# yyyyyxie/textflux

Hardware: AMD Instinct MI355X
Metric: images/sec (whole node), 1024x1024 30-step FLUX-Fill (higher is better)
Workload: dtype bf16

## Files before the change

textflux_amd/csrc/attention_w4.hip:

```cpp
#include <mutex>
#include <type_traits>

#include "common.h"
#include "launch.h"

namespace tfx {

namespace {
constexpr int W4_KV = 64, W4_HD = 128;
constexpr int W4_VT = W4_KV * 256;
constexpr int W4_KROW = 272;
constexpr int W4_KT = W4_KV * W4_KROW;
constexpr int W4_NBUF = 3;
constexpr int W4_KBASE = W4_NBUF * W4_VT;
constexpr int W4_PROW = 132;
__device__ __forceinline__ int w4_part_off(int r, int col) {
  return ((((r >> 5) * 4 + (col >> 5)) * 4 + ((col >> 3) & 3)) * 64 + ((col >> 2) & 1) * 32 + (r & 31)) * 4;
}
constexpr int W4_PART_LM = 256 * 128;
constexpr float W4_THR = 4.0f;
constexpr float W4_BIG = 64.0f;
typedef __attribute__((address_space(3))) s16x4 lds_s16x4;
typedef __attribute__((ext_vector_type(8))) short s16x8;
typedef __attribute__((ext_vector_type(2))) __bf16 bf2_t;
template <int V>
using IC = std::integral_constant<int, V>;
}

constexpr int ATT_LDS_W4 = W4_NBUF * (W4_VT + W4_KT);

#define W4_GAP() __builtin_amdgcn_sched_barrier(0)
#ifndef W4_ABL
#define W4_ABL 0
#endif
#define W4_DRAIN_MFMA()                                                                                                 \
  asm volatile("s_nop 15\n\ts_nop 15\n\ts_nop 15\n\ts_nop 15\n\ts_nop 15\n\ts_nop 15\n\ts_nop 15\n\ts_nop 15\n\t"      \
               "s_nop 15\n\ts_nop 15\n\ts_nop 15\n\ts_nop 15\n\ts_nop 15\n\ts_nop 15\n\ts_nop 15\n\ts_nop 15\n\t"      \
               "s_nop 15\n\ts_nop 15\n\ts_nop 15\n\ts_nop 15\n\ts_nop 15\n\ts_nop 15\n\ts_nop 15\n\ts_nop 15" ::: "memory")

#ifndef W4_NO_TOUCH
#define W4_TOUCH(acc)                                                                  \
  do {                                                                                 \
    const int t_ = __builtin_amdgcn_readfirstlane(__float_as_int((acc)[0]));           \
    asm volatile("" ::"s"(t_));                                                        \
  } while (0)
#else
#define W4_TOUCH(acc) do { } while (0)
#endif

__device__ __forceinline__ void w4_mfma_s0(f32x16& d, const bf16x8& k, const bf16x8& q) {
  f32x16 z;
#pragma unroll
  for (int r = 0; r < 16; ++r) z[r] = 0.f;
  d = __builtin_amdgcn_mfma_f32_32x32x16_bf16(k, q, z, 0, 0, 0);
}
__device__ __forceinline__ void w4_mfma_s(f32x16& d, const bf16x8& k, const bf16x8& q) {
  d = __builtin_amdgcn_mfma_f32_32x32x16_bf16(k, q, d, 0, 0, 0);
}
__device__ __forceinline__ void w4_mfma_o(f32x16& d, const bf16x8& v, const u32x4& p) {
  d = __builtin_amdgcn_mfma_f32_32x32x16_bf16(v, __builtin_bit_cast(bf16x8, p), d, 0, 0, 0);
}
__device__ __forceinline__ void w4_mfma_l(f32x16& d, const bf16x8& ones, const u32x4& p) {
  d = __builtin_amdgcn_mfma_f32_32x32x16_bf16(ones, __builtin_bit_cast(bf16x8, p), d, 0, 0, 0);
}
__device__ __forceinline__ float w4_max7(float a, float b, float c, float d, float e, float f, float g) {
  float r;
  asm("v_max3_f32 %0, %1, %2, %3\n\tv_max3_f32 %0, %0, %4, %5\n\tv_max3_f32 %0, %0, %6, %7"
      : "=&v"(r) : "v"(a), "v"(b), "v"(c), "v"(d), "v"(e), "v"(f), "v"(g));
  return r;
}
__device__ __forceinline__ float w4_max4(float a, float b, float c, float d) {
  float r;
  asm("v_max3_f32 %0, %1, %2, %3\n\tv_max_f32 %0, %0, %4" : "=&v"(r) : "v"(a), "v"(b), "v"(c), "v"(d));
  return r;
}
__device__ __forceinline__ float w4_max(float a, float b) {
  float r;
  asm("v_max_f32 %0, %1, %2" : "=v"(r) : "v"(a), "v"(b));
  return r;
}
__device__ __forceinline__ void w4_dot2c(float& l, uint32_t p) {
  asm volatile("v_dot2c_f32_bf16 %0, 0x3f803f80, %1" : "+v"(l) : "v"(p));
}
__device__ __forceinline__ uint32_t w4_cvt_pk(float lo, float hi) {
  uint32_t r;
  asm volatile("v_cvt_pk_bf16_f32 %0, %1, %2" : "=v"(r) : "v"(lo), "v"(hi));
  return r;
}
#ifdef TFX_BENCH
__device__ unsigned long long* g_w4_timers = nullptr;
#define W4_STAMP(i) do { if (wave == 0) w4_stamp[i] = __builtin_amdgcn_s_memtime(); } while (0)
#else
#define W4_STAMP(i) ((void)0)
#endif
constexpr int W4_SK_MIN = 4;
__host__ __device__ __forceinline__ int w4_sk_bound(int c, int group, int share, int nkv, int total) {
  if (c >= group) return total;
  int p = c * share;
  if (p >= total) return total;
  const int r = p % nkv;
  if (r < W4_SK_MIN) p -= r;
  else if (r > nkv - W4_SK_MIN) p += nkv - r;
  return p < total ? p : total;
}

template <int MODE>
__global__ __launch_bounds__(256, 1) void attn_w4_kernel(const bf16_t* Q, const bf16_t* __restrict__ Kp,
                                                         const bf16_t* __restrict__ Vp, bf16_t* O, int64_t ldq, int64_t ldk,
                                                         int64_t ldv, int64_t ldo, int64_t q_bs, int64_t k_bs, int64_t v_bs,
                                                         int64_t o_bs, int H, int N, int nqb, float scale_log2e, int nfull,
                                                         int nparts, int nsplit, int xsplit, float* part, int T_items, int sk_group,
                                                         int sk_share) {
  extern __shared__ __attribute__((aligned(16))) char smem[];
  constexpr bool LV = MODE == 1 || MODE == 2, LZ = MODE >= 2, NOREF = MODE == 4, FT = LV || NOREF;
  const int tid = threadIdx.x, lane = tid & 63;
  const int wave = __builtin_amdgcn_readfirstlane(tid >> 6);
  const int hi = lane >> 5, l31 = lane & 31;
  int bid = blockIdx.x;
  int kpart = -1, ptile = 0, qblk, h, b;
  int item = 0, item_step = 0, item_end = 0;
  int sk_lo = 0, sk_hi = 0, sk_base = 0, sk_slot0 = 0, sk_u = 0, sk_nunits = 0, sk_nwhole = 0, sk_full = 0, sk_cu = 0, sk_tfirst = 0;
  const int nkv_all = (N + W4_KV - 1) / W4_KV;
  auto sk_unit = [&](int u, int& it, int& ts, int& te) __attribute__((always_inline)) {
    if (u < sk_nwhole) {
      it = sk_base + sk_cu + u * sk_group; ts = 0; te = nkv_all;
    } else {
      const int ti = sk_tfirst + (u - sk_nwhole);
      it = sk_base + sk_full + ti; ts = max(sk_lo - ti * nkv_all, 0); te = min(sk_hi - ti * nkv_all, nkv_all);
    }
  };
  int ts = 0, te = nkv_all;
  if (sk_share > 0) {
    const int L = (bid & 7) * (gridDim.x >> 3) + (bid >> 3);
    const int sample = L / sk_group;
    sk_cu = L - sample * sk_group;
    if (sample >= nfull) return;
    sk_full = (T_items / sk_group) * sk_group;
// ... 850 lines not shown
  if (hipDeviceGetAttribute(&s.cus, hipDeviceAttributeMultiprocessorCount, dev) != hipSuccess || s.cus < 8) s.cus = 256;
  if (hipMalloc((void**)&s.part, (size_t)W4_PART_TILES * 256 * W4_PROW * sizeof(float)) != hipSuccess) {
    (void)hipGetLastError();
    return nullptr;
  }
  g_w4_scr[g_w4_nscr] = s;
  return &g_w4_scr[g_w4_nscr++];
}

int attention_w4_release() {
  std::lock_guard<std::mutex> lk(g_w4_mu);
  if (g_w4_nscr == 0) return 0;
  (void)hipDeviceSynchronize();
  int cur = 0;
  (void)hipGetDevice(&cur);
  for (int i = 0; i < g_w4_nscr; ++i) {
    (void)hipSetDevice(g_w4_scr[i].dev);
    (void)hipDeviceSynchronize();
    (void)hipFree(g_w4_scr[i].part);
  }
  (void)hipSetDevice(cur);
  (void)hipGetLastError();
  g_w4_nscr = 0;
  return 0;
}

int attention_w4_prepare(hipStream_t st) {
  if (!g_w4_split) return 0;
  return w4_scratch(st, true) ? 0 : fail("attention: cannot allocate the tail-split scratch");
}

static int g_w4_streamk = 1;
void set_attention_streamk(int v) { g_w4_streamk = v; }
static int g_w4_persist = 1;
void set_attention_persistent(int v) { g_w4_persist = v; }
static int g_w4_grid() {
  static int grid = 0;
  if (!grid) {
    int dev = 0, cus = 0;
    (void)hipGetDevice(&dev);
    if (hipDeviceGetAttribute(&cus, hipDeviceAttributeMultiprocessorCount, dev) != hipSuccess || cus < 8) cus = 256;
    grid = cus & ~7;
  }
  return grid;
}

#ifdef TFX_BENCH
extern "C" void tfx_bench_attn_timers(unsigned long long* dev) {
  (void)hipMemcpyToSymbol(HIP_SYMBOL(g_w4_timers), &dev, sizeof(dev));
}
#endif

template <int MODE>
static int w4_launch(const AttnArgs& a, hipStream_t st, unsigned grid, int nqb, int nfull, int nparts, int nsplit, int xsplit, float* part,
                     int sk_group, int sk_share) {
  static bool attr_set = false;
  const void* fn = (const void*)attn_w4_kernel<MODE>;
  if (!attr_set) {
    hipFuncAttributes fa;
    if (hipFuncGetAttributes(&fa, fn) != hipSuccess) return fail("attention: no attn_w4_kernel<%d> in this build", MODE);
    (void)hipGetLastError();
    if (fa.localSizeBytes != 0)
      return fail("attention: attn_w4_kernel<%d> spills %zu bytes per lane -- attention_w4.hip must be compiled with "
                  "-mllvm -amdgpu-mfma-vgpr-form", MODE, (size_t)fa.localSizeBytes);
    if (hipFuncSetAttribute(fn, hipFuncAttributeMaxDynamicSharedMemorySize, ATT_LDS_W4 + ((W4_ABL & 256) ? 4096 : 0)) != hipSuccess)
      return fail("attention: cannot raise dynamic LDS limit to %d bytes", ATT_LDS_W4);
    attr_set = true;
  }
  int T_items = 0;
  if (sk_share > 0) {
    T_items = a.H * nqb;
    nfull = a.B;
    grid = (unsigned)g_w4_grid();
  } else if (g_w4_persist && nsplit == 1 && (int)grid > g_w4_grid()) {
    T_items = (int)grid;
    grid = (unsigned)g_w4_grid();
  }
  attn_w4_kernel<MODE><<<grid, 256, ATT_LDS_W4 + ((W4_ABL & 256) ? 4096 : 0), st>>>((const bf16_t*)a.q, (const bf16_t*)a.k, (const bf16_t*)a.v, (bf16_t*)a.o, a.ldq,
                                                       a.ldk, a.ldv, a.ldo, a.q_bstride, a.k_bstride, a.v_bstride, a.o_bstride, a.H,
                                                       a.N, nqb, a.scale * 1.4426950408889634f, nfull, nparts, nsplit, xsplit, part, T_items, sk_group, sk_share);
  return 0;
}

int joint_attention_w4(const AttnArgs& a, hipStream_t st, int mode) {
  const int nqb = (a.N + 255) / 256;
  const int T = a.B * a.H * nqb;
  int nfull = T, nsplit = 1, nparts = 0, xsplit = 0;
  float* part = nullptr;
  if (g_w4_split) {
    hipStreamCaptureStatus cs = hipStreamCaptureStatusNone;
    const bool capturing = !(hipStreamIsCapturing(st, &cs) == hipSuccess && cs == hipStreamCaptureStatusNone);
    (void)hipGetLastError();
    if (const W4Scratch* sc = w4_scratch(st, !capturing)) {
      const int C = sc->cus, tail = T % C, nkv = (a.N + W4_KV - 1) / W4_KV;
      const int m = (tail + a.B - 1) / a.B;
      if (tail && T >= C && m * a.B * 2 <= C + 8 && nkv >= 48 && m < a.H * nqb && m * a.B * 2 <= W4_PART_TILES) {
        xsplit = m; nsplit = 2; nfull = T - m * a.B; nparts = m * a.B * 2; part = sc->part;
      }
    }
  }
  int sk_group = 0, sk_share = 0;
  if (g_w4_streamk && g_w4_persist && nsplit == 1 && a.workspace && a.B <= g_w4_grid()) {
    const int C = g_w4_grid(), nkv = (a.N + W4_KV - 1) / W4_KV, Tp = a.H * nqb, group = C / a.B;
    const int full = (Tp / group) * group, R = Tp - full;
    const int share = R ? (R * nkv + group - 1) / group : 0;
    const int64_t need = (int64_t)2 * a.B * group * 256 * W4_PROW * (int64_t)sizeof(float);
    const float F = 7.f, M = 20.f;
    const float t_whole = (float)(full / group) * ((float)nkv + F);
    const float t_now = t_whole + (float)nkv + F, t_sk = t_whole + (float)share + ((float)share / (float)nkv + 1.f) * F + M;
// ... 30 lines not shown
```

textflux_amd/csrc/capi.cpp:

```cpp
#include "../../include/textflux_hip.h"

#include <cstring>

#include "launch.h"

using namespace tfx;

namespace {

inline hipStream_t S(tfx_stream s) { return (hipStream_t)s; }
inline const uint16_t* bf(const void* p) { return (const uint16_t*)p; }
inline uint16_t* bf(void* p) { return (uint16_t*)p; }

struct Gemm {
  GemmArgs a;
  const tfx_linear* lin;
  Gemm(const void* A, int64_t lda, int64_t abs_, const tfx_linear& l, int64_t ldw, void* C, int64_t ldc, int64_t cbs,
       int M, int N, int K, int batch) : lin(&l) {
    a = GemmArgs();
    a.A = A; a.lda = lda; a.a_bstride = abs_;
    a.W = l.w; a.ldw = ldw; a.bias = l.b;
    a.C = C; a.ldc = ldc; a.c_bstride = cbs;
    a.M = M; a.N = N; a.K = K; a.batch = batch;
    a.epilogue = EPI_BIAS;
// ... 558 lines not shown
int tfx_gather_rows(const void* table, const int64_t* ids, void* out, int64_t n, int32_t D, int64_t vocab, tfx_stream stream) {
  if (!table || !ids || !out) return fail("tfx_gather_rows: null pointer");
  return gather_rows(table, ids, out, n, D, vocab, S(stream));
}
int tfx_add_into_f32(float* x, const void* y, int64_t n, int32_t mode, tfx_stream stream) {
  if (!x || !y) return fail("tfx_add_into_f32: null pointer");
  return add_into_f32(x, y, n, mode, S(stream));
}
int tfx_mul_act(const void* a, int64_t lda, const void* b, int64_t ldb, void* out, int64_t ldo, int64_t rows, int32_t cols,
                int32_t mode, tfx_stream stream) {
  if (!a || !out) return fail("tfx_mul_act: null pointer");
  return mul_act(a, lda, b, ldb, out, ldo, rows, cols, mode, S(stream));
}

int tfx_set_option(const char* name, int value) {
  if (!name) return fail("tfx_set_option: null name");
  if (!std::strcmp(name, "attention_waves")) {
    if (value == 0) { set_attention_waves(0); return 0; }
    if (value != 4 && value != 8 && value != 9 && value != 10 && value != 12 && value != 16 && value != 20 && !(value >= 30 && value <= 34) && value != 40)
      return fail("tfx_set_option: attention_waves must be 4, 8, 9 (128 keys per barrier), 10 / 12 (matrix-pipe softmax, 8 / 4 waves), 16 (ping-pong), 20 (half-tile pipelined), 30 .. 34 (one wave per SIMD, 32x32x16 MFMA: 30 bookkeeping on the matrix pipe -- or no reference at all when the call carries an admissible score bound -- / 31 row sums on the VALU / 32 = 31 + lazy reference offset / 33 = 30 + lazy reference offset / 34 = no reference with a score bound, else 33) or 40 (one wave per SIMD, 16x16x32 MFMA)");
#ifndef TFX_BENCH
    if (value != 30 && value != 34)
      return fail("tfx_set_option: attention_waves %d is a bench-only kernel (libtextflux_hip_bench.so, `make bench`); the product library "
                  "carries 30 (the default) and 34", value);
#endif
    set_attention_waves(value);
    return 0;
  }
  if (!std::strcmp(name, "gemm_group_m")) { set_gemm_group_m(value); return 0; }
  if (!std::strcmp(name, "attention_tail_split")) { set_attention_tail_split(value); return 0; }
  if (!std::strcmp(name, "attention_use_bound")) { set_attention_use_bound(value); return 0; }
  if (!std::strcmp(name, "attention_persistent")) { set_attention_persistent(value); return 0; }
  if (!std::strcmp(name, "attention_streamk")) { set_attention_streamk(value); return 0; }
  if (!std::strcmp(name, "gemm_place")) { set_gemm_place(value); return 0; }
  if (!std::strcmp(name, "gemm_waves")) {
#ifndef TFX_BENCH
    if (value != 8 && value != 0) return fail("tfx_set_option: gemm_waves 4 (gemm4w_kernel) is bench-only (libtextflux_hip_bench.so, `make bench`)");
#endif
    set_gemm_waves(value);
    return 0;
  }
  if (!std::strcmp(name, "gemm_group_streams")) { g_group_streams = value; return 0; }
  if (!std::strcmp(name, "ln_joint")) { g_ln_joint = value; return 0; }
  if (!std::strcmp(name, "ln_prefetch")) { set_ln_prefetch(value); return 0; }
  if (!std::strcmp(name, "fp8_fuse_qkn")) { g_fp8_fuse_qkn = value; return 0; }
  if (!std::strcmp(name, "gemm_splitk")) { set_gemm_splitk(value); return 0; }
  if (!std::strcmp(name, "attention_ablation")) { set_attention_ablation(value); return 0; }
  return fail("tfx_set_option: unknown option '%s'", name);
}

int tfx_debug_attention_timing(void* buf) { set_attention_debug(buf); return 0; }

int tfx_mfma_peak_probe(const void* operands, int64_t operand_bytes, int32_t fp8, int32_t ktiles, double* flops, tfx_stream stream) {
  return mfma_peak_probe(operands, operand_bytes, fp8, ktiles, flops, S(stream));
}

int tfx_prof_enable(int on) { prof_enable(on); return 0; }
int tfx_prof_collect(int kind, double* total_ms, double* total_flops, int* launches) {
  if (kind < 0 || kind > 2) return fail("tfx_prof_collect: kind must be 0 (gemm), 1 (attention) or 2 (fp8 gemm)");
  return prof_collect(kind, total_ms, total_flops, launches);
}

static inline int64_t align256(int64_t v) { return (v + 255) & ~(int64_t)255; }
int tfx_workspace_layout(int32_t B, int32_t Sn, int32_t T, int32_t D, int32_t flags, int64_t* off, int64_t* gemm_ws_bytes) {
  if (B <= 0 || Sn <= 0 || T < 0 || D <= 0 || !off) return fail("tfx_workspace_layout: bad arguments");
  const int64_t N = (int64_t)Sn + T, hid = align256(B * N * D * 2), y = align256(B * N * 7 * (int64_t)D * 2);
// ... 102 lines not shown
```

textflux_amd/csrc/launch.h:

```cpp
#pragma once
#include <hip/hip_runtime.h>
#include <stdint.h>

namespace tfx {

int fail(const char* fmt, ...);
int check_launch(const char* what);
const char* last_error();

void prof_enable(int on);
bool prof_on();
bool prof_on(hipStream_t st);
void prof_begin(int kind, double flops, hipStream_t st);
void prof_end(int kind, hipStream_t st);
int prof_collect(int kind, double* total_ms, double* total_flops, int* launches);

enum Epilogue : int {
  EPI_BIAS = 0,
  EPI_BIAS_GELU = 1,
  EPI_BIAS_GATE_RES = 2,
  EPI_BIAS_RES = 3,
};

struct GemmArgs {
// ... 24 lines not shown
void set_gemm_place(int v);
void set_gemm_waves(int v);
void set_gemm_splitk(int v);
int gemm_bf16(const GemmArgs& a, hipStream_t st);
bool gemm_qkn_ok(const GemmArgs& a);
bool gemm_fp8_qkn_ok(const GemmArgs& a);
int gemm_bf16_variant(const GemmArgs& a, int variant, hipStream_t st);
int gemm_bf16_f32out(const GemmArgs& a, hipStream_t st);
int mfma_peak_probe(const void* operands, int64_t operand_bytes, int fp8, int ktiles, double* flops, hipStream_t st);
int gemm_fp8(const GemmArgs& a, hipStream_t st);
int ln_modulate_fp8(const void* x, void* q8, float* q8_scale, const void* shift, const void* scale, int64_t mod_bstride,
                    int rows_per_batch, int batch, int D, int64_t ldx, int64_t x_bstride, int64_t ldq, int64_t q_bstride,
                    int64_t s_bstride, float eps, hipStream_t st);
int quantize_rows_fp8(const void* x, int64_t ldx, int64_t x_bstride, void* out, int64_t ldo, int64_t o_bstride, float* scale,
                      int64_t s_bstride, int rows, int batch, int K, hipStream_t st);

struct AttnArgs {
  const void* q; const void* k; const void* v; void* o;
  int64_t ldq, ldk, ldv, ldo;
  int64_t q_bstride, k_bstride, v_bstride, o_bstride;
  int B, H, N;
  float scale;
  float score_bound = 0.f;
  void* workspace = nullptr;
  int64_t workspace_bytes = 0;
};
int joint_attention(const AttnArgs& a, hipStream_t st);
int joint_attention_hp(const AttnArgs& a, hipStream_t st);
int joint_attention_w16(const AttnArgs& a, hipStream_t st);
int attention_w4_release();
int attention_w4_prepare(hipStream_t st);
void set_attention_tail_split(int v);
int joint_attention_w4(const AttnArgs& a, hipStream_t st, int mode);
void set_attention_ablation(int a);
void set_attention_use_bound(int v);
int attention_mode_counts(int64_t* counts, int n, int reset);
void attention_note_streamk();
int blend_edge(const void* a, int64_t a_bs, int64_t a_ts, int64_t a_us, void* b, int64_t b_bs, int64_t b_ts, int64_t b_us, int batch,
               int extent, int len, int C, hipStream_t st);
int gate_residual(const void* x, int64_t ldx, int64_t x_bs, const void* gate, int64_t gate_bs, const void* res, int64_t ldr, int64_t r_bs,
                  void* out, int64_t ldo, int64_t o_bs, int rows, int batch, int D, hipStream_t st);
void set_attention_streamk(int v);
void set_attention_persistent(int v);
void set_attention_debug(void* p);
void set_attention_waves(int nw);

int groupnorm_silu_nhwc(const void* x, void* out, const void* gamma, const void* beta, float* stats_ws, int B,
                        int64_t HW, int C, int groups, float eps, bool silu, hipStream_t st);
void set_ln_prefetch(int v);
int ln_modulate_split(const void* x, void* out, const void* shift, const void* scale, const void* shift2, const void* scale2,
                      int split_row, int64_t mod_bstride, int rows_per_batch, int batch, int D, int64_t ldx, int64_t x_bstride, int64_t ldo,
                      int64_t o_bstride, float eps, hipStream_t st);
int ln_modulate(const void* x, void* out, const void* shift, const void* scale, int64_t mod_bstride,
                int rows_per_batch, int batch, int D, int64_t ldx, int64_t x_bstride, int64_t ldo,
                int64_t o_bstride, float eps, hipStream_t st);
int layernorm_affine(const void* x, void* out, const void* gamma, const void* beta, int64_t rows, int D, int64_t ldx, int64_t ldo,
                     float eps, hipStream_t st);
int rmsnorm_rope(void* buf, int64_t ld, int64_t bstride, int q_off, int k_off, int H, int Ntok, int T, int B,
                 const void* wq_img, const void* wk_img, const void* wq_txt, const void* wk_txt, const float* cosT,
                 const float* sinT, float eps, hipStream_t st);
int sched_step(bool amo, const void* v, void* x, void* xin, int64_t ldxin, int C, int64_t rows, const float* coef,
               const int* step_ptr, int step, const float* noise, hipStream_t st);
int timestep_embedding(const float* t, void* out, int n, hipStream_t st);
int silu_bf16(const void* a, void* out, int64_t n, hipStream_t st);
int add_bf16(const void* a, const void* b, void* out, int64_t n, hipStream_t st);
int scatter_cols(const void* src, void* dst, int64_t rows, int C, int64_t ld, int col0, hipStream_t st);
// ... 32 lines not shown
```

Baseline: 0.5871.

## Add register-resident fixed-reference attention kernel for the no-rescale mode

Adds a separate attention kernel that is used for MODE 4 (the no-reference-max path) when there is no tail split. It keeps a dedicated software-pipelined schedule: raw v_exp with no running max or rescale, row sums accumulated with v_add instead of an MFMA or dot2c, next-item Q prefetched into registers, and K/V staged through registers into a triple LDS buffer. Shared constants and helpers move to a common header. The aim is fewer instructions per tile in the exp/sum stage and better MFMA/VALU interleaving, at the cost of a second large hand-scheduled kernel to maintain.

```diff
diff --git a/textflux_amd/csrc/attention_rf.hip b/textflux_amd/csrc/attention_rf.hip
--- /dev/null
+++ b/textflux_amd/csrc/attention_rf.hip
@@ -0,0 +1,438 @@
+#include "attention_w4.h"
+#include "launch.h"
+
+namespace tfx {
+
+#ifdef TFX_BENCH
+__device__ unsigned long long* g_rf_timers = nullptr;
+#define RF_STAMP(i) do { if (wave == 0) rf_stamp[i] = __builtin_amdgcn_s_memtime(); } while (0)
+#else
+#define RF_STAMP(i) ((void)0)
+#endif
+
+__device__ __forceinline__ float rf_exp(float x) {
+  asm volatile("v_exp_f32 %0, %0" : "+v"(x));
+  return x;
+}
+__device__ __forceinline__ void rf_add(float& l, float x) { asm volatile("v_add_f32 %0, %0, %1" : "+v"(l) : "v"(x)); }
+
+__global__ __launch_bounds__(256, 1) void attn_rf_kernel(const bf16_t* Q, const bf16_t* __restrict__ Kp, const bf16_t* __restrict__ Vp,
+                                                         bf16_t* O, int64_t ldq, int64_t ldk, int64_t ldv, int64_t ldo, int64_t q_bs,
+                                                         int64_t k_bs, int64_t v_bs, int64_t o_bs, int H, int N, int nqb, float scale_log2e,
+                                                         int nfull, float* part, int T_items, int sk_group, int sk_share) {
+  extern __shared__ __attribute__((aligned(16))) char smem[];
+  const int tid = threadIdx.x, lane = tid & 63;
+  const int wave = __builtin_amdgcn_readfirstlane(tid >> 6);
+  const int hi = lane >> 5, l31 = lane & 31;
+  int bid = blockIdx.x;
+  int qblk, h, b;
+  int item = 0, item_step = 0, item_end = 0;
+  int sk_lo = 0, sk_hi = 0, sk_base = 0, sk_slot0 = 0, sk_u = 0, sk_nunits = 0, sk_nwhole = 0, sk_full = 0, sk_cu = 0, sk_tfirst = 0;
+  const int nkv_all = (N + W4_KV - 1) / W4_KV;
+  auto sk_unit = [&](int u, int& it, int& ts, int& te) __attribute__((always_inline)) {
+    if (u < sk_nwhole) {
+      it = sk_base + sk_cu + u * sk_group; ts = 0; te = nkv_all;
+    } else {
+      const int ti = sk_tfirst + (u - sk_nwhole);
+      it = sk_base + sk_full + ti; ts = max(sk_lo - ti * nkv_all, 0); te = min(sk_hi - ti * nkv_all, nkv_all);
+    }
+  };
+  int ts = 0, te = nkv_all;
+  if (sk_share > 0) {
+    const int L = (bid & 7) * (gridDim.x >> 3) + (bid >> 3);
+    const int sample = L / sk_group;
+    sk_cu = L - sample * sk_group;
+    if (sample >= nfull) return;
+    sk_full = (T_items / sk_group) * sk_group;
+    sk_nwhole = sk_full / sk_group;
+    const int total = (T_items - sk_full) * nkv_all;
+    sk_lo = w4_sk_bound(sk_cu, sk_group, sk_share, nkv_all, total);
+    sk_hi = w4_sk_bound(sk_cu + 1, sk_group, sk_share, nkv_all, total);
+    sk_tfirst = sk_lo / nkv_all;
+    sk_nunits = sk_nwhole + (sk_hi > sk_lo ? (sk_hi - 1) / nkv_all - sk_tfirst + 1 : 0);
+    if (sk_nunits == 0) return;
+    sk_base = sample * T_items;
+    sk_slot0 = 2 * L;
+    sk_unit(0, item, ts, te);
+  } else if (T_items > 0) {
+    const int nwg = gridDim.x, q = T_items >> 3, r = T_items & 7, xcd = bid & 7, slot = bid >> 3;
+    const int xs = xcd < r ? xcd * (q + 1) : r * (q + 1) + (xcd - r) * q, xc = q + (xcd < r ? 1 : 0);
+    if (slot >= xc) return;
+    item = xs + slot;
+    item_step = nwg >> 3;
+    item_end = xs + xc;
+  } else {
+    const int nwg = gridDim.x, q = nwg >> 3, r = nwg & 7, xcd = bid & 7, k = bid >> 3;
+    item = (xcd < r ? xcd * (q + 1) : r * (q + 1) + (xcd - r) * q) + k;
+  }
+  qblk = item % nqb;
+  h = (item / nqb) % H;
+  b = item / (nqb * H);
+  bf16x8 qn[2][8];
+  bool have_pref = false;
+  u32x4 kreg[4], vreg[4];
+#ifdef TFX_BENCH
+  unsigned long long rf_stamp[4] = {0, 0, 0, 0}, rf_sum[4] = {0, 0, 0, 0};
+#endif
+  for (;;) {
+  RF_STAMP(0);
+  bool has_next = item + item_step < item_end;
+  int item2 = item + item_step, ts2 = 0;
+  if (sk_share > 0) {
+    int te2;
+    has_next = sk_u + 1 < sk_nunits;
+    if (has_next) sk_unit(sk_u + 1, item2, ts2, te2);
+  }
+  const int qblk2 = item2 % nqb, h2 = (item2 / nqb) % H, b2 = item2 / (nqb * H);
+  const bf16_t* Qb = Q + b * q_bs + h * W4_HD;
+  const bf16_t* Kb = Kp + b * k_bs + h * W4_HD;
+  const bf16_t* Vb = Vp + b * v_bs + h * W4_HD;
+  bf16_t* Ob = O + b * o_bs + h * W4_HD;
+  int Nk = N;
+  int pslot = -1;
+  if (sk_share > 0) {
+    if (ts > 0) pslot = sk_slot0;
+    else if (te < nkv_all) pslot = sk_slot0 + 1;
+    Nk = min(N, te * W4_KV) - ts * W4_KV;
+    Kb += (int64_t)ts * W4_KV * ldk;
+    Vb += (int64_t)ts * W4_KV * ldv;
+  }
+
+  bf16x8 qf[2][8];
+#pragma unroll
+  for (int qb = 0; qb < 2; ++qb) {
+    const int qrow = qblk * 256 + wave * 64 + qb * 32 + l31;
+    const int rc = qrow < N ? qrow : N - 1;
+    if (have_pref) {
+#pragma unroll
+      for (int s = 0; s < 8; ++s) qf[qb][s] = qn[qb][s];
+    } else {
+#pragma unroll
+      for (int s = 0; s < 8; ++s) qf[qb][s] = *reinterpret_cast<const bf16x8*>(Qb + (int64_t)rc * ldq + s * 16 + hi * 8);
+    }
+  }
+  auto load_qn = [&]() __attribute__((always_inline)) {
+    const bf16_t* Qb2 = Q + b2 * q_bs + h2 * W4_HD;
+#pragma unroll
+    for (int qb = 0; qb < 2; ++qb) {
+      const int r2 = qblk2 * 256 + wave * 64 + qb * 32 + l31;
+      const int rc = r2 < N ? r2 : N - 1;
+#pragma unroll
+      for (int s = 0; s < 8; ++s) qn[qb][s] = *reinterpret_cast<const bf16x8*>(Qb2 + (int64_t)rc * ldq + s * 16 + hi * 8);
+    }
+  };
+  __builtin_amdgcn_sched_barrier(0);
+  auto convert_q = [&]() __attribute__((always_inline)) {
+#pragma unroll
+    for (int qb = 0; qb < 2; ++qb)
+#pragma unroll
+      for (int s = 0; s < 8; ++s) {
+#pragma unroll
+        for (int e = 0; e < 8; ++e) qf[qb][s][e] = (__bf16)((float)qf[qb][s][e] * scale_log2e);
+        asm volatile("" : "+a"(qf[qb][s]));
+      }
+  };
+
+  const int nkv = (Nk + W4_KV - 1) / W4_KV;
+  const int ldk2 = (int)ldk * 2, ldv2 = (int)ldv * 2;
+  const auto rsK = __builtin_amdgcn_make_buffer_rsrc((void*)Kb, 0, (int)((uint32_t)(Nk - 1) * (uint32_t)ldk2 + 256u), 0x00020000);
+  const auto rsV = __builtin_amdgcn_make_buffer_rsrc((void*)Vb, 0, (int)((uint32_t)(Nk - 1) * (uint32_t)ldv2 + 256u), 0x00020000);
+  const auto rsK2 = __builtin_amdgcn_make_buffer_rsrc((void*)(Kp + b2 * k_bs + h2 * W4_HD + (int64_t)ts2 * W4_KV * ldk), 0,
+                                                      (int)((uint32_t)(N - 1 - ts2 * W4_KV) * (uint32_t)ldk2 + 256u), 0x00020000);
+  const auto rsV2 = __builtin_amdgcn_make_buffer_rsrc((void*)(Vp + b2 * v_bs + h2 * W4_HD + (int64_t)ts2 * W4_KV * ldv), 0,
+                                                      (int)((uint32_t)(N - 1 - ts2 * W4_KV) * (uint32_t)ldv2 + 256u), 0x00020000);
+  auto rsKs = rsK, rsVs = rsV;
+  auto load_piece = [&](int j, int ko, int vo, auto Ic, bool k_side) __attribute__((always_inline)) {
+    constexpr int i = decltype(Ic)::value;
+    if (k_side)
+      kreg[i] = __builtin_bit_cast(u32x4, __builtin_amdgcn_raw_buffer_load_b128(rsKs, ko, (j * W4_KV + 16 * i) * ldk2, 0));
+    else
+      vreg[i] = __builtin_bit_cast(u32x4, __builtin_amdgcn_raw_buffer_load_b128(rsVs, vo, (j * W4_KV + 16 * i) * ldv2, 0));
+  };
+  auto stage_offsets = [&](int& ko, int& vo) __attribute__((always_inline)) {
+    int te_ = tid;
+    asm volatile("" : "+v"(te_));
+    ko = (int)__umul24(te_ >> 4, ldk2) + (te_ & 15) * 16;
+    vo = (int)__umul24(te_ >> 4, ldv2) + (te_ & 15) * 16;
+  };
+  auto load_tile = [&](int j) __attribute__((always_inline)) {
+    int ko, vo;
+    stage_offsets(ko, vo);
+    load_piece(j, ko, vo, IC<0>{}, true); load_piece(j, ko, vo, IC<0>{}, false); load_piece(j, ko, vo, IC<1>{}, true); load_piece(j, ko, vo, IC<1>{}, false);
+    load_piece(j, ko, vo, IC<2>{}, true); load_piece(j, ko, vo, IC<2>{}, false); load_piece(j, ko, vo, IC<3>{}, true); load_piece(j, ko, vo, IC<3>{}, false);
+  };
+  auto write_piece = [&](int buf, auto Ic, bool k_side) __attribute__((always_inline)) {
+    constexpr int i = decltype(Ic)::value;
+    const int kr = tid >> 4, ch = tid & 15;
+    if (k_side)
+      *reinterpret_cast<u32x4*>(smem + W4_KBASE + buf * W4_KT + kr * W4_KROW + ch * 16 + i * 16 * W4_KROW) = kreg[i];
+    else
+      *reinterpret_cast<u32x4*>(smem + buf * W4_VT + kr * 256 + ((((ch >> 2) ^ (kr & 3)) << 6) | ((ch & 3) << 4)) + i * 16 * 256) = vreg[i];
+  };
+  auto write_tile = [&](int buf) __attribute__((always_inline)) {
+    write_piece(buf, IC<0>{}, true); write_piece(buf, IC<0>{}, false); write_piece(buf, IC<1>{}, true); write_piece(buf, IC<1>{}, false);
+    write_piece(buf, IC<2>{}, true); write_piece(buf, IC<2>{}, false); write_piece(buf, IC<3>{}, true); write_piece(buf, IC<3>{}, false);
+  };
+  const char* rK = smem + W4_KBASE + l31 * W4_KROW + hi * 16;
+  const int vi = lane & 15;
+  const char* rV[4];
+#pragma unroll
+  for (int db = 0; db < 4; ++db)
+    rV[db] = smem + (4 * hi + (vi >> 2)) * 256 + 32 * ((lane >> 4) & 1) + (vi & 3) * 8 + ((db ^ ((vi >> 2) & 3)) << 6);
+  auto kread = [&](int koff, int s) __attribute__((always_inline)) -> bf16x8 {
+    return *reinterpret_cast<const bf16x8*>(rK + koff + s * 32);
+  };
+  auto vread = [&](int voff, int ks, int db) __attribute__((always_inline)) -> bf16x8 {
+    const char* va = rV[db] + voff + ks * 16 * 256;
+    const s16x4 lo = __builtin_amdgcn_ds_read_tr16_b64_v4i16((lds_s16x4*)(va));
+    const s16x4 hi4 = __builtin_amdgcn_ds_read_tr16_b64_v4i16((lds_s16x4*)(va + 8 * 256));
+    return __builtin_bit_cast(bf16x8, (s16x8)__builtin_shufflevector(lo, hi4, 0, 1, 2, 3, 4, 5, 6, 7));
+  };
+
+  f32x16 o[2][4], sc[2];
+#pragma unroll
+  for (int qb = 0; qb < 2; ++qb)
+#pragma unroll
+    for (int r = 0; r < 16; ++r)
+#pragma unroll
+      for (int db = 0; db < 4; ++db) o[qb][db][r] = 0.f;
+  bf16x8 kf[8], vf[2][4];
+  u32x4 pf[2][2];
+  float lsum[2] = {0.f, 0.f};
+
+  if (!have_pref) load_tile(0);
+  u32x4 k1[4], v1[4];
+  {
+    int ko, vo;
+    stage_offsets(ko, vo);
+#pragma unroll
+    for (int i = 0; i < 4; ++i) {
+      k1[i] = __builtin_bit_cast(u32x4, __builtin_amdgcn_raw_buffer_load_b128(rsK, ko, (W4_KV + 16 * i) * ldk2, 0));
+      v1[i] = __builtin_bit_cast(u32x4, __builtin_amdgcn_raw_buffer_load_b128(rsV, vo, (W4_KV + 16 * i) * ldv2, 0));
+    }
+  }
+  __builtin_amdgcn_sched_barrier(0);
+  convert_q();
+  __builtin_amdgcn_sched_barrier(0);
+  write_tile(0);
+  load_tile(2);
+  {
+    const int kr = tid >> 4, ch = tid & 15;
+#pragma unroll
+    for (int i = 0; i < 4; ++i) {
+      *reinterpret_cast<u32x4*>(smem + W4_KBASE + W4_KT + kr * W4_KROW + ch * 16 + i * 16 * W4_KROW) = k1[i];
+      *reinterpret_cast<u32x4*>(smem + W4_VT + kr * 256 + ((((ch >> 2) ^ (kr & 3)) << 6) | ((ch & 3) << 4)) + i * 16 * 256) = v1[i];
+    }
+  }
+  __syncthreads();
+#pragma unroll
+  for (int s = 0; s < 8; ++s) kf[s] = kread(0, s);
+  W4_GAP();
+  w4_mfma_s0(sc[0], kf[0], qf[0][0]);
+#pragma unroll
+  for (int s = 1; s < 8; ++s) w4_mfma_s(sc[0], kf[s], qf[0][s]);
+  W4_GAP();
+
+  auto step = [&](auto QBc, auto PVc, auto KNc, auto VNc, auto STGc, int jst, bool rag, int kb_abs) __attribute__((always_inline)) {
+    constexpr int QB = decltype(QBc)::value, OQ = 1 - QB;
+    constexpr bool EVEN = QB == 0, PV = decltype(PVc)::value != 0;
+    constexpr int KN = decltype(KNc)::value, VN = decltype(VNc)::value, STG = decltype(STGc)::value;
+    f32x16& cur = sc[QB];
+    f32x16& nxt = sc[OQ];
+    if (__builtin_expect_with_probability(rag, 0, 1.0)) {
+      int kbase = kb_abs + 4 * hi;
+      asm volatile("" : "+v"(kbase));
+#pragma unroll
+      for (int r = 0; r < 16; ++r)
+        if (kbase + (r & 3) + 8 * (r >> 2) >= Nk) cur[r] = -INFINITY;
+    }
+    auto S = [&](auto Ic) __attribute__((always_inline)) {
+      constexpr int i = decltype(Ic)::value;
+      if constexpr (i == 1) w4_mfma_s0(nxt, kf[0], qf[OQ][0]);
+      else w4_mfma_s(nxt, kf[i - 1], qf[OQ][i - 1]);
+      if constexpr (EVEN && i >= 2) kf[i - 2] = kread(KN, i - 2);
+    };
+    auto PL = [&](auto Ic) __attribute__((always_inline)) {
+      constexpr int i = decltype(Ic)::value, ks = i / 4, db = i % 4;
+      if constexpr (PV) w4_mfma_o(o[OQ][db], vf[ks][db], pf[OQ][ks]);
+      if constexpr (EVEN && i >= 1) vf[(i - 1) / 4][(i - 1) % 4] = vread(VN, (i - 1) / 4, (i - 1) % 4);
+    };
+    auto RL = [&]() __attribute__((always_inline)) {
+      if constexpr (EVEN) {
+        vf[1][3] = vread(VN, 1, 3);
+        kf[7] = kread(KN, 7);
+      }
+    };
+    auto E = [&](auto Ic) __attribute__((always_inline)) { cur[decltype(Ic)::value] = rf_exp(cur[decltype(Ic)::value]); };
+    auto A = [&](auto Ic) __attribute__((always_inline)) { rf_add(lsum[QB], cur[decltype(Ic)::value]); };
+    auto C = [&](auto Ic) __attribute__((always_inline)) {
+      constexpr int c = decltype(Ic)::value;
+      pf[QB][c >> 2][c & 3] = w4_cvt_pk(cur[2 * c], cur[2 * c + 1]);
+    };
+    int stg_ko = 0, stg_vo = 0;
+    if constexpr (STG & 3) stage_offsets(stg_ko, stg_vo);
+    auto G = [&](auto Ic) __attribute__((always_inline)) {
+      constexpr int n = decltype(Ic)::value;
+      if constexpr (STG & 3) {
+        constexpr bool is_w = n == 0 || n == 1 || n == 3 || n == 5;
+        constexpr int g = 4 * ((STG & 3) - 1) + (n < 2 ? n : is_w ? (n + 1) / 2 : n == 7 ? 3 : n / 2 - 1);
+        if constexpr (is_w) write_piece(STG >> 2, IC<g / 2>{}, (g & 1) == 0);
+        else load_piece(jst, stg_ko, stg_vo, IC<g / 2>{}, (g & 1) == 0);
+      }
+    };
+    S(IC<1>{}); W4_TOUCH(cur); E(IC<0>{});
+    W4_GAP();
+    PL(IC<0>{}); E(IC<1>{}); A(IC<0>{}); G(IC<0>{});
+    W4_GAP();
+    S(IC<2>{}); E(IC<2>{}); A(IC<1>{}); C(IC<0>{});
+    W4_GAP();
+    PL(IC<1>{}); E(IC<3>{}); A(IC<2>{}); G(IC<1>{});
+    W4_GAP();
+    S(IC<3>{}); E(IC<4>{}); A(IC<3>{}); C(IC<1>{});
+    W4_GAP();
+    PL(IC<2>{}); E(IC<5>{}); A(IC<4>{}); G(IC<2>{});
+    W4_GAP();
+    S(IC<4>{}); E(IC<6>{}); A(IC<5>{}); C(IC<2>{});
+    W4_GAP();
+    PL(IC<3>{}); E(IC<7>{}); A(IC<6>{}); G(IC<3>{});
+    W4_GAP();
+    S(IC<5>{}); E(IC<8>{}); A(IC<7>{}); C(IC<3>{});
+    W4_GAP();
+    PL(IC<4>{}); E(IC<9>{}); A(IC<8>{}); G(IC<4>{});
+    W4_GAP();
+    S(IC<6>{}); E(IC<10>{}); A(IC<9>{}); C(IC<4>{});
+    W4_GAP();
+    PL(IC<5>{}); E(IC<11>{}); A(IC<10>{}); G(IC<5>{});
+    W4_GAP();
+    S(IC<7>{}); E(IC<12>{}); A(IC<11>{}); C(IC<5>{});
+    W4_GAP();
+    S(IC<8>{}); E(IC<13>{}); A(IC<12>{});
+#ifdef W4_HAZARD_SELFTEST
+    { float t_; asm volatile("v_add_f32 %0, %1, %2" : "=v"(t_) : "v"(nxt[0]), "v"(nxt[1])); asm volatile("" ::"v"(t_)); }
+#endif
+    W4_GAP();
+    PL(IC<6>{}); E(IC<14>{}); A(IC<13>{}); C(IC<6>{}); G(IC<6>{});
+    W4_GAP();
+    PL(IC<7>{}); E(IC<15>{}); A(IC<14>{}); C(IC<7>{}); A(IC<15>{}); G(IC<7>{}); RL();
+    W4_GAP();
+  };
+
+  const int j_rag = (Nk & (W4_KV - 1)) ? nkv - 1 : -1;
+  auto tile = [&](int j, auto Bc, auto FIRSTc) __attribute__((always_inline)) {
+    constexpr int B = decltype(Bc)::value, NB = (B + 1) % 3, WB = (B + 2) % 3;
+    constexpr int FIRST = decltype(FIRSTc)::value;
+    const bool rag = j == j_rag;
+    step(IC<0>{}, IC<!FIRST>{}, IC<B * W4_KT + 32 * W4_KROW>{}, IC<B * W4_VT>{}, IC<0>{}, 0, rag, j * W4_KV);
+    step(IC<1>{}, IC<1>{}, IC<0>{}, IC<0>{}, IC<1 + 4 * WB>{}, j + 3, rag, j * W4_KV);
+    step(IC<0>{}, IC<1>{}, IC<NB * W4_KT>{}, IC<B * W4_VT + 2 * 16 * 256>{}, IC<0>{}, 0, rag, j * W4_KV + 32);
+    step(IC<1>{}, IC<1>{}, IC<0>{}, IC<0>{}, IC<2 + 4 * WB>{}, j + 3, rag, j * W4_KV + 32);
+    __builtin_amdgcn_sched_barrier(0);
+    asm volatile("s_waitcnt lgkmcnt(0)" ::: "memory");
+    __builtin_amdgcn_s_barrier();
+    __builtin_amdgcn_sched_barrier(0);
+  };
+  RF_STAMP(1);
+  tile(0, IC<0>{}, IC<1>{});
+  for (int j = 1; j < nkv; j += 3) {
+    tile(j, IC<1>{}, IC<0>{});
+    if (j + 1 < nkv) tile(j + 1, IC<2>{}, IC<0>{});
+    if (j + 2 < nkv) tile(j + 2, IC<0>{}, IC<0>{});
+  }
+  RF_STAMP(2);
+  asm volatile("s_waitcnt vmcnt(0)" ::: "memory");
+  if (has_next) load_qn();
+#pragma unroll
+  for (int ks = 0; ks < 2; ++ks)
+#pragma unroll
+    for (int db = 0; db < 4; ++db) w4_mfma_o(o[1][db], vf[ks][db], pf[1][ks]);
+  float ltot[2];
+#pragma unroll
+  for (int qb = 0; qb < 2; ++qb) ltot[qb] = lsum[qb] + __shfl_xor(lsum[qb], 32, 64);
+
+  if (pslot >= 0) {
+    float* pp = part + (int64_t)pslot * (256 * W4_PROW);
+#pragma unroll
+    for (int qb = 0; qb < 2; ++qb) {
+      float* pr = pp + (wave * 2 + qb) * (16 * 256) + lane * 4;
+#pragma unroll
+      for (int db = 0; db < 4; ++db)
+#pragma unroll
+        for (int qd = 0; qd < 4; ++qd)
+          *reinterpret_cast<f32x4*>(pr + (db * 4 + qd) * 256) =
+              f32x4{o[qb][db][qd * 4 + 0], o[qb][db][qd * 4 + 1], o[qb][db][qd * 4 + 2], o[qb][db][qd * 4 + 3]};
+      if (hi == 0) *reinterpret_cast<float2*>(pp + W4_PART_LM + (wave * 64 + qb * 32 + l31) * 2) = float2{ltot[qb], 0.f};
+    }
+  } else {
+  constexpr int OROW = 272;
+  char* ot = smem + wave * (64 * OROW);
+#pragma unroll
+  for (int qb = 0; qb < 2; ++qb) {
+    const float inv = 1.0f / ltot[qb];
+    char* orow = ot + (qb * 32 + l31) * OROW + 8 * hi;
+#pragma unroll
+    for (int db = 0; db < 4; ++db)
+#pragma unroll
+      for (int qd = 0; qd < 4; ++qd) {
+        u32x2 w;
+        w[0] = pack_bf2(o[qb][db][qd * 4 + 0] * inv, o[qb][db][qd * 4 + 1] * inv);
+        w[1] = pack_bf2(o[qb][db][qd * 4 + 2] * inv, o[qb][db][qd * 4 + 3] * inv);
+        *reinterpret_cast<u32x2*>(orow + db * 64 + qd * 16) = w;
+      }
+  }
+  __builtin_amdgcn_fence(__ATOMIC_RELEASE, "wavefront");
+  asm volatile("s_waitcnt lgkmcnt(0)" ::: "memory");
+  const int row0 = qblk * 256 + wave * 64;
+#pragma unroll
+  for (int i = 0; i < 16; ++i) {
+    const int c = lane + 64 * i, row = c >> 4, ch = c & 15;
+    const u32x4 v = *reinterpret_cast<const u32x4*>(ot + row * OROW + ch * 16);
+    if (row0 + row < N) *reinterpret_cast<u32x4*>(Ob + (int64_t)(row0 + row) * ldo + ch * 8) = v;
+  }
+  }
+#ifdef TFX_BENCH
+  RF_STAMP(3);
+  rf_sum[0] += rf_stamp[1] - rf_stamp[0]; rf_sum[1] += rf_stamp[2] - rf_stamp[1]; rf_sum[2] += rf_stamp[3] - rf_stamp[2]; rf_sum[3] += 1;
+  if (!has_next && g_rf_timers && tid == 0)
+    for (int i = 0; i < 4; ++i) atomicAdd(g_rf_timers + i, rf_sum[i]);
+#endif
+  if (!has_next) break;
+  rsKs = rsK2;
+  rsVs = rsV2;
+  load_tile(0);
+  item = item2; b = b2; h = h2; qblk = qblk2;
+  if (sk_share > 0) { ++sk_u; int it_; sk_unit(sk_u, it_, ts, te); }
+  have_pref = true;
+  __builtin_amdgcn_sched_barrier(0);
+  asm volatile("s_waitcnt lgkmcnt(0)" ::: "memory");
+  __builtin_amdgcn_s_barrier();
+  __builtin_amdgcn_sched_barrier(0);
+  }
+}
+
+#ifdef TFX_BENCH
+void attn_rf_bench_timers(unsigned long long* dev) {
+  (void)hipMemcpyToSymbol(HIP_SYMBOL(g_rf_timers), &dev, sizeof(dev));
+}
+#endif
+
+int attn_rf_launch(const AttnArgs& a, hipStream_t st, unsigned grid, int nqb, int nfull, float* part, int T_items, int sk_group, int sk_share) {
+  static bool attr_set = false;
+  const void* fn = (const void*)attn_rf_kernel;
+  if (!attr_set) {
+    hipFuncAttributes fa;
+    if (hipFuncGetAttributes(&fa, fn) != hipSuccess) return fail("attention: no attn_rf_kernel in this build");
+    (void)hipGetLastError();
+    if (fa.localSizeBytes != 0)
+      return fail("attention: attn_rf_kernel spills %zu bytes per lane -- attention_rf.hip must be compiled with -mllvm -amdgpu-mfma-vgpr-form",
+                  (size_t)fa.localSizeBytes);
+    if (hipFuncSetAttribute(fn, hipFuncAttributeMaxDynamicSharedMemorySize, ATT_LDS_W4) != hipSuccess)
+      return fail("attention: cannot raise dynamic LDS limit to %d bytes", ATT_LDS_W4);
+    attr_set = true;
+  }
+  attn_rf_kernel<<<grid, 256, ATT_LDS_W4, st>>>((const bf16_t*)a.q, (const bf16_t*)a.k, (const bf16_t*)a.v, (bf16_t*)a.o, a.ldq, a.ldk, a.ldv,
+                                               a.ldo, a.q_bstride, a.k_bstride, a.v_bstride, a.o_bstride, a.H, a.N, nqb,
+                                               a.scale * 1.4426950408889634f, nfull, part, T_items, sk_group, sk_share);
+  return 0;
+}
+
+}
diff --git a/textflux_amd/csrc/attention_w4.h b/textflux_amd/csrc/attention_w4.h
--- /dev/null
+++ b/textflux_amd/csrc/attention_w4.h
@@ -0,0 +1,70 @@
+#pragma once
+#include <type_traits>
+
+#include "common.h"
+
+namespace tfx {
+
+namespace {
+constexpr int W4_KV = 64, W4_HD = 128;
+constexpr int W4_VT = W4_KV * 256;
+constexpr int W4_KROW = 272;
+constexpr int W4_KT = W4_KV * W4_KROW;
+constexpr int W4_NBUF = 3;
+constexpr int W4_KBASE = W4_NBUF * W4_VT;
+constexpr int W4_PROW = 132;
+__device__ __forceinline__ int w4_part_off(int r, int col) {
+  return ((((r >> 5) * 4 + (col >> 5)) * 4 + ((col >> 3) & 3)) * 64 + ((col >> 2) & 1) * 32 + (r & 31)) * 4;
+}
+constexpr int W4_PART_LM = 256 * 128;
+typedef __attribute__((address_space(3))) s16x4 lds_s16x4;
+typedef __attribute__((ext_vector_type(8))) short s16x8;
+typedef __attribute__((ext_vector_type(2))) __bf16 bf2_t;
+template <int V>
+using IC = std::integral_constant<int, V>;
+}
+
+constexpr int ATT_LDS_W4 = W4_NBUF * (W4_VT + W4_KT);
+
+#define W4_GAP() __builtin_amdgcn_sched_barrier(0)
+
+#ifndef W4_NO_TOUCH
+#define W4_TOUCH(acc)                                                                  \
+  do {                                                                                 \
+    const int t_ = __builtin_amdgcn_readfirstlane(__float_as_int((acc)[0]));           \
+    asm volatile("" ::"s"(t_));                                                        \
+  } while (0)
+#else
+#define W4_TOUCH(acc) do { } while (0)
+#endif
+
+__device__ __forceinline__ void w4_mfma_s0(f32x16& d, const bf16x8& k, const bf16x8& q) {
+  f32x16 z;
+#pragma unroll
+  for (int r = 0; r < 16; ++r) z[r] = 0.f;
+  d = __builtin_amdgcn_mfma_f32_32x32x16_bf16(k, q, z, 0, 0, 0);
+}
+__device__ __forceinline__ void w4_mfma_s(f32x16& d, const bf16x8& k, const bf16x8& q) {
+  d = __builtin_amdgcn_mfma_f32_32x32x16_bf16(k, q, d, 0, 0, 0);
+}
+__device__ __forceinline__ void w4_mfma_o(f32x16& d, const bf16x8& v, const u32x4& p) {
+  d = __builtin_amdgcn_mfma_f32_32x32x16_bf16(v, __builtin_bit_cast(bf16x8, p), d, 0, 0, 0);
+}
+__device__ __forceinline__ uint32_t w4_cvt_pk(float lo, float hi) {
+  uint32_t r;
+  asm volatile("v_cvt_pk_bf16_f32 %0, %1, %2" : "=v"(r) : "v"(lo), "v"(hi));
+  return r;
+}
+
+constexpr int W4_SK_MIN = 4;
+__host__ __device__ __forceinline__ int w4_sk_bound(int c, int group, int share, int nkv, int total) {
+  if (c >= group) return total;
+  int p = c * share;
+  if (p >= total) return total;
+  const int r = p % nkv;
+  if (r < W4_SK_MIN) p -= r;
+  else if (r > nkv - W4_SK_MIN) p += nkv - r;
+  return p < total ? p : total;
+}
+
+}
diff --git a/textflux_amd/csrc/attention_w4.hip b/textflux_amd/csrc/attention_w4.hip
--- a/textflux_amd/csrc/attention_w4.hip
+++ b/textflux_amd/csrc/attention_w4.hip
@@ -1,35 +1,15 @@
 #include <mutex>
-#include <type_traits>
-
-#include "common.h"
+
+#include "attention_w4.h"
 #include "launch.h"
 
 namespace tfx {
 
 namespace {
-constexpr int W4_KV = 64, W4_HD = 128;
-constexpr int W4_VT = W4_KV * 256;
-constexpr int W4_KROW = 272;
-constexpr int W4_KT = W4_KV * W4_KROW;
-constexpr int W4_NBUF = 3;
-constexpr int W4_KBASE = W4_NBUF * W4_VT;
-constexpr int W4_PROW = 132;
-__device__ __forceinline__ int w4_part_off(int r, int col) {
-  return ((((r >> 5) * 4 + (col >> 5)) * 4 + ((col >> 3) & 3)) * 64 + ((col >> 2) & 1) * 32 + (r & 31)) * 4;
-}
-constexpr int W4_PART_LM = 256 * 128;
 constexpr float W4_THR = 4.0f;
 constexpr float W4_BIG = 64.0f;
-typedef __attribute__((address_space(3))) s16x4 lds_s16x4;
-typedef __attribute__((ext_vector_type(8))) short s16x8;
-typedef __attribute__((ext_vector_type(2))) __bf16 bf2_t;
-template <int V>
-using IC = std::integral_constant<int, V>;
-}
-
-constexpr int ATT_LDS_W4 = W4_NBUF * (W4_VT + W4_KT);
-
-#define W4_GAP() __builtin_amdgcn_sched_barrier(0)
+}
+
 #ifndef W4_ABL
 #define W4_ABL 0
 #endif
@@ -38,28 +18,6 @@
                "s_nop 15\n\ts_nop 15\n\ts_nop 15\n\ts_nop 15\n\ts_nop 15\n\ts_nop 15\n\ts_nop 15\n\ts_nop 15\n\t"      \
                "s_nop 15\n\ts_nop 15\n\ts_nop 15\n\ts_nop 15\n\ts_nop 15\n\ts_nop 15\n\ts_nop 15\n\ts_nop 15" ::: "memory")
 
-#ifndef W4_NO_TOUCH
-#define W4_TOUCH(acc)                                                                  \
-  do {                                                                                 \
-    const int t_ = __builtin_amdgcn_readfirstlane(__float_as_int((acc)[0]));           \
-    asm volatile("" ::"s"(t_));                                                        \
-  } while (0)
-#else
-#define W4_TOUCH(acc) do { } while (0)
-#endif
-
-__device__ __forceinline__ void w4_mfma_s0(f32x16& d, const bf16x8& k, const bf16x8& q) {
-  f32x16 z;
-#pragma unroll
-  for (int r = 0; r < 16; ++r) z[r] = 0.f;
-  d = __builtin_amdgcn_mfma_f32_32x32x16_bf16(k, q, z, 0, 0, 0);
-}
-__device__ __forceinline__ void w4_mfma_s(f32x16& d, const bf16x8& k, const bf16x8& q) {
-  d = __builtin_amdgcn_mfma_f32_32x32x16_bf16(k, q, d, 0, 0, 0);
-}
-__device__ __forceinline__ void w4_mfma_o(f32x16& d, const bf16x8& v, const u32x4& p) {
-  d = __builtin_amdgcn_mfma_f32_32x32x16_bf16(v, __builtin_bit_cast(bf16x8, p), d, 0, 0, 0);
-}
 __device__ __forceinline__ void w4_mfma_l(f32x16& d, const bf16x8& ones, const u32x4& p) {
   d = __builtin_amdgcn_mfma_f32_32x32x16_bf16(ones, __builtin_bit_cast(bf16x8, p), d, 0, 0, 0);
 }
@@ -82,27 +40,12 @@
 __device__ __forceinline__ void w4_dot2c(float& l, uint32_t p) {
   asm volatile("v_dot2c_f32_bf16 %0, 0x3f803f80, %1" : "+v"(l) : "v"(p));
 }
-__device__ __forceinline__ uint32_t w4_cvt_pk(float lo, float hi) {
-  uint32_t r;
-  asm volatile("v_cvt_pk_bf16_f32 %0, %1, %2" : "=v"(r) : "v"(lo), "v"(hi));
-  return r;
-}
 #ifdef TFX_BENCH
 __device__ unsigned long long* g_w4_timers = nullptr;
 #define W4_STAMP(i) do { if (wave == 0) w4_stamp[i] = __builtin_amdgcn_s_memtime(); } while (0)
 #else
 #define W4_STAMP(i) ((void)0)
 #endif
-constexpr int W4_SK_MIN = 4;
-__host__ __device__ __forceinline__ int w4_sk_bound(int c, int group, int share, int nkv, int total) {
-  if (c >= group) return total;
-  int p = c * share;
-  if (p >= total) return total;
-  const int r = p % nkv;
-  if (r < W4_SK_MIN) p -= r;
-  else if (r > nkv - W4_SK_MIN) p += nkv - r;
-  return p < total ? p : total;
-}
 
 template <int MODE>
 __global__ __launch_bounds__(256, 1) void attn_w4_kernel(const bf16_t* Q, const bf16_t* __restrict__ Kp,
@@ -1019,6 +962,8 @@
 
 static int g_w4_streamk = 1;
 void set_attention_streamk(int v) { g_w4_streamk = v; }
+static int g_w4_rf = 1;
+void set_attention_rf(int v) { g_w4_rf = v; }
 static int g_w4_persist = 1;
 void set_attention_persistent(int v) { g_w4_persist = v; }
 static int g_w4_grid() {
@@ -1035,12 +980,23 @@
 #ifdef TFX_BENCH
 extern "C" void tfx_bench_attn_timers(unsigned long long* dev) {
   (void)hipMemcpyToSymbol(HIP_SYMBOL(g_w4_timers), &dev, sizeof(dev));
+  attn_rf_bench_timers(dev);
 }
 #endif
 
 template <int MODE>
 static int w4_launch(const AttnArgs& a, hipStream_t st, unsigned grid, int nqb, int nfull, int nparts, int nsplit, int xsplit, float* part,
                      int sk_group, int sk_share) {
+  int T_items = 0;
+  if (sk_share > 0) {
+    T_items = a.H * nqb;
+    nfull = a.B;
+    grid = (unsigned)g_w4_grid();
+  } else if (g_w4_persist && nsplit == 1 && (int)grid > g_w4_grid()) {
+    T_items = (int)grid;
+    grid = (unsigned)g_w4_grid();
+  }
+  if (MODE == 4 && g_w4_rf && nsplit == 1) return attn_rf_launch(a, st, grid, nqb, nfull, part, T_items, sk_group, sk_share);
   static bool attr_set = false;
   const void* fn = (const void*)attn_w4_kernel<MODE>;
   if (!attr_set) {
@@ -1053,15 +1009,6 @@
     if (hipFuncSetAttribute(fn, hipFuncAttributeMaxDynamicSharedMemorySize, ATT_LDS_W4 + ((W4_ABL & 256) ? 4096 : 0)) != hipSuccess)
       return fail("attention: cannot raise dynamic LDS limit to %d bytes", ATT_LDS_W4);
     attr_set = true;
-  }
-  int T_items = 0;
-  if (sk_share > 0) {
-    T_items = a.H * nqb;
-    nfull = a.B;
-    grid = (unsigned)g_w4_grid();
-  } else if (g_w4_persist && nsplit == 1 && (int)grid > g_w4_grid()) {
-    T_items = (int)grid;
-    grid = (unsigned)g_w4_grid();
   }
   attn_w4_kernel<MODE><<<grid, 256, ATT_LDS_W4 + ((W4_ABL & 256) ? 4096 : 0), st>>>((const bf16_t*)a.q, (const bf16_t*)a.k, (const bf16_t*)a.v, (bf16_t*)a.o, a.ldq,
                                                        a.ldk, a.ldv, a.ldo, a.q_bstride, a.k_bstride, a.v_bstride, a.o_bstride, a.H,
diff --git a/textflux_amd/csrc/capi.cpp b/textflux_amd/csrc/capi.cpp
--- a/textflux_amd/csrc/capi.cpp
+++ b/textflux_amd/csrc/capi.cpp
@@ -614,6 +614,7 @@
   if (!std::strcmp(name, "attention_use_bound")) { set_attention_use_bound(value); return 0; }
   if (!std::strcmp(name, "attention_persistent")) { set_attention_persistent(value); return 0; }
   if (!std::strcmp(name, "attention_streamk")) { set_attention_streamk(value); return 0; }
+  if (!std::strcmp(name, "attention_rf")) { set_attention_rf(value); return 0; }
   if (!std::strcmp(name, "gemm_place")) { set_gemm_place(value); return 0; }
   if (!std::strcmp(name, "gemm_waves")) {
 #ifndef TFX_BENCH
diff --git a/textflux_amd/csrc/launch.h b/textflux_amd/csrc/launch.h
--- a/textflux_amd/csrc/launch.h
+++ b/textflux_amd/csrc/launch.h
@@ -80,6 +80,12 @@
 int attention_w4_prepare(hipStream_t st);
 void set_attention_tail_split(int v);
 int joint_attention_w4(const AttnArgs& a, hipStream_t st, int mode);
+int attn_rf_launch(const AttnArgs& a, hipStream_t st, unsigned grid, int nqb, int nfull, float* part, int T_items, int sk_group,
+                   int sk_share);
+void set_attention_rf(int v);
+#ifdef TFX_BENCH
+void attn_rf_bench_timers(unsigned long long* dev);
+#endif
 void set_attention_ablation(int a);
 void set_attention_use_bound(int v);
 int attention_mode_counts(int64_t* counts, int n, int reset);
```

Result: faster. 0.5954 (median of 6 runs) (+1.4%).
